# TGAC/KAT

Hardware: AMD Instinct MI355X
Metric: k-mers/sec (whole node) for kat comp reads-vs-assembly k=27 (higher is better)
Workload: dtype u64

## Files before the change

### kat_amd/csrc/kg_count.hip

```cpp
#include "kg_host.hpp"
#include "kg_ingest.hpp"
#include "kg_kernels.hpp"
#include "kg_partition.hpp"
#include "kg_partition_wide.hpp"
#include "kg_wide.hpp"

#include <condition_variable>
#include <deque>
#include <mutex>
#include <thread>


static const uint64_t g_test_sweep_thr = hook("KATGPU_TEST_SWEEP_THR") ? strtoull(hook("KATGPU_TEST_SWEEP_THR"), nullptr, 10) : 0;
static const uint64_t g_test_max_starts = hook("KATGPU_TEST_MAX_STARTS") ? strtoull(hook("KATGPU_TEST_MAX_STARTS"), nullptr, 10) : 0;

static int maybe_sweep(katgpu_table* t, uint64_t next_starts) {
    katgpu_ctx* c = t->ctx;
    if (t->dev().cbits) return KATGPU_OK;
    const uint64_t limit = g_test_sweep_thr ? 2 * g_test_sweep_thr - 1 : 0xFFFFFFFFULL;
    if (t->count_bound + t->unchecked_adds + next_starts <= limit) return KATGPU_OK;
    const uint32_t thr = g_test_sweep_thr ? (uint32_t)g_test_sweep_thr : 0x80000000u;
    unsigned long long* scratch = (unsigned long long*)&t->dev().ctrs[CTR_SCRATCH];
    HIPCHK(c, hipMemsetAsync(scratch, 0, sizeof(uint64_t), c->stream));
    {
        ScopedTimer tm(c, KATGPU_K_REGROW, t->dev().cap);
        hipLaunchKernelGGL(k_sweep, dim3(grid_for(c, t->dev().cap, 256, 8)), dim3(256), 0, c->stream, t->dev(), thr, scratch);
    }
    uint64_t mx = 0;
    HIPCHK(c, hipMemcpyAsync(&mx, scratch, sizeof mx, hipMemcpyDeviceToHost, c->stream));
    HIPCHK(c, hipStreamSynchronize(c->stream));
    t->count_bound = mx;
    t->unchecked_adds = 0;
    return KATGPU_OK;
}

static int launch_count(katgpu_table* t, const uint8_t* dev_bases, size_t n) {
    katgpu_ctx* c = t->ctx;
    if (n < t->dev().k) return KATGPU_OK;
    if (t->dev().keys_b) {
        const uint64_t n_chunks = (n + WIDE_CHUNK_STARTS - 1) / WIDE_CHUNK_STARTS;
        const int grid = (int)std::min<uint64_t>(n_chunks, (uint64_t)c->n_cu * 4);
        ScopedTimer tm(c, KATGPU_K_COUNT, n);
        if ((reinterpret_cast<uintptr_t>(dev_bases) & 15) == 0)
            hipLaunchKernelGGL((k_count<true, true>), dim3(grid), dim3(COUNT_BLOCK), 0, c->stream, t->dev(), dev_bases, (uint64_t)n, n_chunks);
        else
            hipLaunchKernelGGL((k_count<false, true>), dim3(grid), dim3(COUNT_BLOCK), 0, c->stream, t->dev(), dev_bases, (uint64_t)n, n_chunks);
        HIPCHK(c, hipGetLastError());
        return KATGPU_OK;
    }
    int src = maybe_sweep(t, n);
    if (src) return src;
    t->unchecked_adds += n;
    const uint64_t n_chunks = (n + CHUNK_STARTS - 1) / CHUNK_STARTS;
    const int grid = (int)std::min<uint64_t>(n_chunks, (uint64_t)c->n_cu * c->count_blocks_per_cu);
    ScopedTimer tm(c, KATGPU_K_COUNT, n);
    if ((reinterpret_cast<uintptr_t>(dev_bases) & 15) == 0)
        hipLaunchKernelGGL(k_count<true>, dim3(grid), dim3(COUNT_BLOCK), 0, c->stream, t->dev(), dev_bases, (uint64_t)n, n_chunks);
    else
        hipLaunchKernelGGL(k_count<false>, dim3(grid), dim3(COUNT_BLOCK), 0, c->stream, t->dev(), dev_bases, (uint64_t)n, n_chunks);
    HIPCHK(c, hipGetLastError());
    return KATGPU_OK;
}



static const uint64_t g_part_min_starts = getenv("KATGPU_PART_MIN_STARTS") ? strtoull(getenv("KATGPU_PART_MIN_STARTS"), nullptr, 10) : (32ULL << 20);
static const uint64_t g_test_round_items = hook("KATGPU_TEST_ROUND_ITEMS") ? strtoull(hook("KATGPU_TEST_ROUND_ITEMS"), nullptr, 10) : 0;
static const double g_arena_fraction = getenv("KATGPU_ARENA_FRACTION") ? std::min(0.95, std::max(0.05, atof(getenv("KATGPU_ARENA_FRACTION")))) : 0.85;
static const uint32_t g_p1_wgs = hook("KATGPU_P1_WGS") ? std::max<uint32_t>(1, (uint32_t)strtoul(hook("KATGPU_P1_WGS"), nullptr, 10)) : 3;
static const uint32_t g_test_l1_cpb = hook("KATGPU_TEST_L1_CPB") ? (uint32_t)strtoul(hook("KATGPU_TEST_L1_CPB"), nullptr, 10) : 0;
static const bool g_l1_lean = hook_u64("KATGPU_L1_LEAN", 1) != 0;
static const uint32_t g_l1_fast = hook("KATGPU_L1_FAST") ? (uint32_t)strtoul(hook("KATGPU_L1_FAST"), nullptr, 10) : 1;
static const uint32_t g_p2_fast = hook("KATGPU_P2_FAST") ? (uint32_t)strtoul(hook("KATGPU_P2_FAST"), nullptr, 10) : 1;
static const uint64_t g_test_p2_ovf_cap = hook("KATGPU_TEST_P2_OVF_CAP") ? strtoull(hook("KATGPU_TEST_P2_OVF_CAP"), nullptr, 10) : 0;
static const uint32_t g_test_spill_mod = hook("KATGPU_TEST_SPILL_MOD") ? (uint32_t)strtoul(hook("KATGPU_TEST_SPILL_MOD"), nullptr, 10) : 0;
static const uint64_t g_test_ap_seg = hook_u64("KATGPU_TEST_AP_SEG", 0) & ~3ULL;
static const uint32_t g_apply_per_cu = (uint32_t)hook_u64("KATGPU_APPLY_PER_CU", 0);
static const bool g_l1b_stamp = hook_u64("KATGPU_L1B_STAMP", 0) != 0;
static const bool g_p2x_stamp = hook_u64("KATGPU_P2X_STAMP", 0) != 0;
static const bool g_p2_stamp = hook_u64("KATGPU_P2_STAMP", 0) != 0;
static const bool g_apply_stamp = hook_u64("KATGPU_APPLY_STAMP", 0) != 0;

static bool part_geometry(const DevTable& d, PartGeom* g) {
    g->R = d.n_regions; g->S = d.region_slots; g->P1 = d.p1; g->P2 = d.p2; g->l2 = d.l2;
    g->b_lo = 0; g->b_hi = d.p1;
    g->pl = place_make(d.k, d.p1, d.n1, d.l2);
    g->hb = l2_hi_bytes(g->pl.rb);
    g->hb1 = l2_hi_bytes(g->pl.n1);
    g->cbits = d.cbits;
    if (d.cbits && g->hb > 2) g->hb = 2;
    return d.k <= 32 && g->pl.rb <= 63  && g->P1 <= MAX_PARTS && g->P2 <= MAX_PARTS && g->S % 4 == 0 && g->S >= 64 && g->S <= AP2_MAX_SLOTS;
}
static double l2_items_per_l1_item(uint32_t hb) { return 1 + 1.0 / 16 + 2.0 * MAX_PARTS / l2_tile_items(hb); }
static const uint32_t g_test_pass_buckets = hook("KATGPU_TEST_PASS_BUCKETS") ? (uint32_t)strtoul(hook("KATGPU_TEST_PASS_BUCKETS"), nullptr, 10) : 0;
static uint32_t pass_buckets(uint32_t p1, uint32_t n_cu) {
    if (g_test_pass_buckets) return std::max<uint32_t>(1, std::min(p1, g_test_pass_buckets));
    return n_cu && p1 > n_cu && p1 % n_cu == 0 ? n_cu : p1;
}
static double arena_bytes_per_item(uint32_t hb, uint32_t passes) { return 8.0 * (1 + 1.0 / 24) + l2_bytes_per_item(hb) * (1 + 1.0 / 24) * l2_items_per_l1_item(hb) / passes + 0.25 + 0.02; }

static const bool g_test_grow_nomem = hook("KATGPU_TEST_GROW_NOMEM") != nullptr;

static void insert_keys(katgpu_table* t, const void* keys, uint64_t n, size_t key_bytes) {
    katgpu_ctx* c = t->ctx;
    ScopedTimer tm(c, KATGPU_K_COUNT, n);
    if (key_bytes == 16) hipLaunchKernelGGL(k_insert_keys_w, dim3(grid_for(c, n, 256, 6)), dim3(256), 0, c->stream, t->dev(), (const u64x2*)keys, n);
    else hipLaunchKernelGGL(k_insert_keys, dim3(grid_for(c, n, 256, 6)), dim3(256), 0, c->stream, t->dev(), (const uint64_t*)keys, n);
}
typedef std::vector<std::pair<const void*, uint64_t>> KeyLists;
static int grow_beside_arena(katgpu_table* t, uint64_t incoming, uint64_t min_cap, const KeyLists& stash, size_t key_bytes, bool* arena_lost) {
    uint64_t n_stash = 0;
    for (auto& l : stash) n_stash += l.second;
    katgpu_ctx* c = t->ctx;
    auto grow = [&]() -> int {
        if (min_cap > t->dev().cap) {
            if (t->disable_grow) return fail(c, KATGPU_ERR_TABLE_FULL, "Hash full");
            uint64_t nc = t->dev().cap; while (nc < min_cap) nc *= 2;
            return regrow(t, nc);
        }
        return ensure_room(t, incoming);
    };
    *arena_lost = false;
    int rc = g_test_grow_nomem ? KATGPU_ERR_NOMEM : grow();
    if (rc != KATGPU_ERR_NOMEM) return rc;
    (void)hipGetLastError();
    std::vector<uint8_t> host;
    if (n_stash) {
        try { host.resize(n_stash * key_bytes); } catch (...) { return fail(c, KATGPU_ERR_NOMEM, "no host memory to park %llu spilled k-mers", (unsigned long long)n_stash); }
        uint64_t at = 0;
        for (auto& l : stash) { HIPCHK(c, hipMemcpy(host.data() + at * key_bytes, l.first, l.second * key_bytes, hipMemcpyDeviceToHost)); at += l.second; }
    }
    HIPCHK(c, hipStreamSynchronize(c->stream));
    release_arena(c);
    *arena_lost = true;
    if (g_trace) fprintf(stderr, "[katgpu] growth beside the partition arena failed: arena released, %llu keys parked on the host\n", (unsigned long long)n_stash);
    rc = grow();
    if (rc) return rc;
    if (n_stash) {
        const size_t chunk = std::min<size_t>(n_stash, ((size_t)256 << 20) / key_bytes);
        uint8_t* d = nullptr;
        HIPCHK(c, pool_alloc(c, (void**)&d, chunk * key_bytes));
        for (size_t i = 0; i < n_stash && rc == KATGPU_OK; i += chunk) {
            const size_t m = std::min(chunk, (size_t)n_stash - i);
            if (hipMemcpyAsync(d, host.data() + i * key_bytes, m * key_bytes, hipMemcpyHostToDevice, c->stream) != hipSuccess) { rc = fail(c, KATGPU_ERR_DEVICE, "spill upload"); break; }
            insert_keys(t, d, m, key_bytes);
            if (hipStreamSynchronize(c->stream) != hipSuccess) rc = fail(c, KATGPU_ERR_DEVICE, "spill insert");
        }
        pool_release(c, d);
    }
    return rc;
}

static int ensure_arena(katgpu_ctx* c, size_t small_bytes, size_t item_bytes, size_t want_items, size_t want_bytes, const char* note, bool* usable) {
    *usable = false;
    if (c->arena_limit) want_bytes = std::min(want_bytes, std::max(c->arena_limit, small_bytes + item_bytes * ((size_t)64 << 20)));
    if (c->arena_bytes < want_bytes) {
        size_t free_b = 0, total_b = 0;
        HIPCHK(c, hipMemGetInfo(&free_b, &total_b));
        free_b += c->arena_bytes;
        const size_t bytes = std::min<size_t>(want_bytes, (size_t)(g_arena_fraction * (double)free_b));
        if (bytes > c->arena_bytes + c->arena_bytes / 2 || c->arena_bytes < small_bytes + item_bytes * std::min<size_t>(want_items, (size_t)64 << 20)) {
            if (c->arena) { HIPCHK(c, hipFree(c->arena)); c->arena = nullptr; c->arena_bytes = 0; }
            if (!g_test_round_items && bytes < small_bytes + item_bytes * ((size_t)1 << 20)) return KATGPU_OK;
            const double t_ar = now_ms();
            if (hipMalloc((void**)&c->arena, bytes) != hipSuccess) { (void)hipGetLastError(); c->arena = nullptr; return KATGPU_OK; }
            c->arena_bytes = bytes;
            if (g_trace) fprintf(stderr, "[katgpu +%.0f ms] partition arena of %.1f GB%s: %.0f ms\n", since_load(), bytes / 1e9, note, now_ms() - t_ar);
        }
    }
    *usable = true;
    return KATGPU_OK;
}
struct ArenaBusy { katgpu_ctx* c; explicit ArenaBusy(katgpu_ctx* c_) : c(c_) { c->arena_busy = true; } ~ArenaBusy() { c->arena_busy = false; } };
template <typename T> static T* carve(uint8_t*& a, size_t bytes) { T* p = (T*)a; a += align_up(bytes, 256); return p; }

constexpr size_t LDS_BYTES = 160 * 1024, LDS_GRANULE = 1280;
template <typename K, typename... Args>
static int launch_lds(katgpu_ctx* c, K kern, dim3 grid, dim3 block, size_t lds, size_t ceiling, Args... args) {
    if (!c->lds_attr.count(reinterpret_cast<const void*>(kern))) {
        HIPCHK(c, hipFuncSetAttribute(reinterpret_cast<const void*>(kern), hipFuncAttributeMaxDynamicSharedMemorySize, (int)ceiling));
        c->lds_attr.insert(reinterpret_cast<const void*>(kern));
    }
    hipLaunchKernelGGL(kern, grid, block, lds, c->stream, args...);
    return KATGPU_OK;
}

struct StampLine { const char* head; int n_shown, n_sum; const char* phase[9];  int digits; };
static const StampLine STAMPS_L1B = {"[katgpu] level-1 (blocks) stamps (wave 0 of every workgroup, cycles summed):", 9, 9,
    {" codes %.*f %%", "  blocks out %.*f %%", " (+ barrier %.*f %%)", "  sweep %.*f %%", " (+ %.*f %%)", "  per bucket %.*f %%", " (+ %.*f %%)", "  placing %.*f %%", " (+ %.*f %%)"}, 1};
static const StampLine STAMPS_P2X = {"[katgpu] level-2 (blocks in, blocks out) stamps (wave 0 of every workgroup, cycles summed):", 7, 9,
    {" wait for the tile %.*f %%", " (+ barrier %.*f %%)", "  ranking + blocks out %.*f %%", " (+ %.*f %%)", "  per sub-bucket %.*f %%", " (+ %.*f %%)", "  placing %.*f %%"}, 1};
static const StampLine STAMPS_P2 = {"[katgpu] level-2 stamps (lane 0 of every workgroup, cycles summed):", 5, 5,
    {" wait for the tile %.*f %%", "  digit + rank %.*f %%", "  scan %.*f %%", "  staging %.*f %%", "  copy-out %.*f %%"}, 0};
constexpr int STAMP_AT_APPLY = 8, STAMP_AT = 16;
template <typename Launch>
static int with_stamps(katgpu_ctx* c, unsigned long long* dev, int n, const StampLine* line, Launch launch) {
    unsigned long long st[10];
    HIPCHK(c, hipMemsetAsync(dev, 0, n * sizeof(unsigned long long), c->stream));
    int rc = launch(dev);
    if (rc) return rc;
    HIPCHK(c, hipMemcpyAsync(st, dev, n * sizeof(unsigned long long), hipMemcpyDeviceToHost, c->stream));
    HIPCHK(c, hipStreamSynchronize(c->stream));
    double tot = line ? 0 : (double)(st[0] + st[1] + st[3] + st[4]);
    if (!line && st[5])
        fprintf(stderr, "[katgpu] apply stamps (wave 0 of every workgroup, cycles summed): fill %.3g (%.0f %%)  walk %.3g (%.0f %%; drains %.0f %% of the walk)  barrier + sweep %.3g (%.0f %%)  write-back %.3g (%.0f %%); %llu regions, %.1f chunks per wave and region, %.0f cycles per region\n",
                (double)st[0], 100 * st[0] / tot, (double)st[1], 100 * st[1] / tot, 100.0 * st[2] / std::max(1.0, (double)st[1]), (double)st[3], 100 * st[3] / tot, (double)st[4], 100 * st[4] / tot, st[5], (double)st[6] / st[5], tot / st[5]);
    if (!line || !st[n - 1]) return KATGPU_OK;
    for (int i = 0; i < line->n_sum; ++i) tot += (double)st[i];
    char buf[768];
    int at = snprintf(buf, sizeof buf, "%s", line->head);
    for (int i = 0; i < line->n_shown; ++i) at += snprintf(buf + at, sizeof buf - at, line->phase[i], line->digits, 100 * st[i] / tot);
    fprintf(stderr, "%s; %llu tiles, %.0f cycles per tile\n", buf, st[n - 1], tot / st[n - 1]);
    return KATGPU_OK;
}

struct ApplyLaunch {
    katgpu_table* t; const PartGeom& g; const uint64_t* off2; const uint8_t* l2_buf; uint64_t* spill_buf; unsigned long long* spill_n; const uint32_t* run_len; const uint64_t* bucket_end;
    dim3 grid; size_t lds; uint32_t qcap; uint64_t seg_len; uint32_t zero_fill;
};
template <int B, int KP, int HB, bool INL, bool HK, bool PF, int NR, bool STAMP = false>
static int apply_pk(const ApplyLaunch& a) {
    return launch_lds(a.t->ctx, k_p3_apply_pk<B, KP, HB, INL, HK, PF, NR, STAMP>, a.grid, dim3(B), a.lds, LDS_BYTES - 256, a.t->dv, a.g, a.off2, a.l2_buf, a.spill_buf, a.spill_n, a.run_len, a.bucket_end,
                      a.qcap, a.seg_len, g_test_spill_mod, a.zero_fill);
}
template <int HB>
static int apply_pk_shape(const ApplyLaunch& a, uint32_t blk, bool fresh, bool hooked) {
    if (hooked) return apply_pk<1024, 5, HB, false, true, true, 3>(a);
    if (blk == 1024) return fresh ? apply_pk<1024, 5, HB, true, false, true, 3>(a) : apply_pk<1024, 5, HB, false, false, true, 2>(a);
    if (a.g.S <= 4096) return fresh ? apply_pk<512, 4, HB, true, false, true, 3>(a) : apply_pk<512, 4, HB, false, false, true, 2>(a);
    if (HB == 1 && g_apply_stamp && !fresh)
        return with_stamps(a.t->ctx, a.spill_n + STAMP_AT_APPLY, 7, nullptr, [&](unsigned long long*) { return apply_pk<512, 10, 1, false, false, false, 2, true>(a); });
    return fresh ? apply_pk<512, 10, HB, true, false, false, 3>(a) : apply_pk<512, 10, HB, false, false, false, 2>(a);
}
template <int B, int KP, int HB, bool INL, int QC, bool HK>
static int apply_kv12(const ApplyLaunch& a) {
    return launch_lds(a.t->ctx, k_p3_apply2<B, KP, 4, 3, HB, false, INL, true, QC, HK>, a.grid, dim3(B), a.lds, LDS_BYTES - 256, a.t->dev(), a.g, a.off2, a.l2_buf, a.spill_buf, a.spill_n, a.run_len, a.bucket_end,
                      (unsigned long long*)nullptr, g_test_spill_mod, a.seg_len);
}
template <int HB>
static int apply_kv12_shape(const ApplyLaunch& a, uint32_t blk, bool big, bool fresh, bool hooked) {
    if (hooked) return apply_kv12<1024, 5, HB, false, AP2_QCAP_BIG, true>(a);
    if (blk == 512 && a.g.S <= 2048) return fresh ? apply_kv12<512, 2, HB, true, AP2_QCAP, false>(a) : apply_kv12<512, 2, HB, false, AP2_QCAP, false>(a);
    if (blk == 512) return fresh ? apply_kv12<512, 4, HB, true, AP2_QCAP, false>(a) : apply_kv12<512, 4, HB, false, AP2_QCAP, false>(a);
    if (big) return fresh ? apply_kv12<1024, 5, HB, true, AP2_QCAP_BIG, false>(a) : apply_kv12<1024, 5, HB, false, AP2_QCAP_BIG, false>(a);
    return fresh ? apply_kv12<1024, 4, HB, true, AP2_QCAP, false>(a) : apply_kv12<1024, 4, HB, false, AP2_QCAP, false>(a);
}
static int launch_apply(katgpu_table* t, const PartGeom& g, const uint64_t* off2, const uint8_t* l2_buf, uint64_t* spill_buf, unsigned long long* spill_n,
                        const uint32_t* run_len, const uint64_t* bucket_end) {
    katgpu_ctx* c = t->ctx;
    const uint32_t n_cu = (uint32_t)c->n_cu, regions = (g.b_hi - g.b_lo) * g.P2;
    const bool fresh = t->distinct == 0;
    const bool hooked = g_test_spill_mod != 0;
    ApplyLaunch a{t, g, off2, l2_buf, spill_buf, spill_n, run_len, bucket_end, dim3(1), 0, 0, 0, 0};
    int rc = KATGPU_OK;
    if (g.cbits) {
        const size_t region_b = (size_t)g.S * 8;
        auto room = [&](uint32_t wgs) -> long { return (long)(LDS_BYTES / wgs / LDS_GRANULE * LDS_GRANULE) - 64 - (long)region_b; };
        uint32_t per_cu = 4;
        auto min_q = [&](uint32_t wgs) -> long { return 8L * 8 * (wgs == 2 ? 72 : 96); };
        while (per_cu > 1 && room(per_cu) < min_q(per_cu)) --per_cu;
        if (g_apply_per_cu) per_cu = std::min(per_cu, g_apply_per_cu);
        uint32_t blk = per_cu == 1 ? 1024 : 512;
        if (hooked) { blk = 1024; per_cu = 1; }
        per_cu = std::min<uint32_t>(per_cu, 2048 / blk);
        const uint32_t nw = blk / 64;
        while (per_cu > 1 && room(per_cu) < (long)(nw * 72 * 8)) --per_cu;
        a.qcap = (uint32_t)std::min<long>(256, room(per_cu) / (long)(nw * 8));
        if (a.qcap < 72) return fail(c, KATGPU_ERR_DEVICE, "a region of %u packed slots leaves no room for the apply kernel's queues", g.S);
        a.lds = region_b + (size_t)nw * a.qcap * 8;
        const uint64_t seg_cap = (pk_half(g.cbits) - 1) & ~3ULL;
        a.seg_len = g_test_ap_seg ? std::min<uint64_t>(g_test_ap_seg, seg_cap) : std::min<uint64_t>(AP2_SEGMENT, seg_cap);
        a.grid = dim3(std::min<uint32_t>(regions, n_cu * per_cu));
        const uint64_t r_lo = (uint64_t)g.b_lo * g.P2, r_hi = (uint64_t)g.b_hi * g.P2;
        if (t->zero_from != ~0ULL) { if (t->zero_from == r_lo) a.zero_fill = 1; else t->zero_rest(); }
        switch (g.hb) {
        case 0: rc = apply_pk_shape<0>(a, blk, fresh, hooked); break;
        case 1: rc = apply_pk_shape<1>(a, blk, fresh, hooked); break;
        case 2: rc = apply_pk_shape<2>(a, blk, fresh, hooked); break;
        default: return fail(c, KATGPU_ERR_DEVICE, "packed apply: item width %u", g.hb);
        }
        if (rc) return rc;
        HIPCHK(c, hipGetLastError());
        if (a.zero_fill) t->zero_from = r_hi >= t->dv.n_regions ? ~0ULL : r_hi;
        return KATGPU_OK;
    }
    const uint32_t blk = hooked ? 1024 : (g.S <= 4096 ? 512 : 1024);
    const bool big = g.S > 8192 || hooked;
    a.lds = (size_t)g.S * 12 + (size_t)(blk / 64) * (big ? AP2_QCAP_BIG : AP2_QCAP) * 12;
    const uint32_t per_cu = (uint32_t)std::max<size_t>(1, std::min<size_t>(LDS_BYTES / (a.lds + 512), 2048 / blk));
    a.grid = dim3(std::min<uint32_t>(regions, n_cu * per_cu));
    a.seg_len = g_test_ap_seg ? std::min<uint64_t>(g_test_ap_seg, AP2_SEGMENT) : AP2_SEGMENT;
    switch (g.hb) {
    case 0: rc = apply_kv12_shape<0>(a, blk, big, fresh, hooked); break;
    case 1: rc = apply_kv12_shape<1>(a, blk, big, fresh, hooked); break;
    case 2: rc = apply_kv12_shape<2>(a, blk, big, fresh, hooked); break;
    case 4: rc = apply_kv12_shape<4>(a, blk, big, fresh, hooked); break;
    }
    if (rc) return rc;
    HIPCHK(c, hipGetLastError());
    return KATGPU_OK;
}

constexpr size_t SEG_PAD = 64;
struct PartArena {
    uint32_t hb, passes; double per_item; size_t fixed_l1, small_bytes;
    uint32_t* hist1; uint64_t* offs; uint64_t* l1_off; uint64_t* off2; uint32_t* cnt2; uint64_t* bend; unsigned long long* spill_n; unsigned long long* ovf_n;
    uint8_t* l1_buf;
    uint8_t* l2_buf;
    uint64_t* ovf_buf; uint64_t ovf_cap;
    size_t round_items, l1_items, l2_items;
    PartArena(const PartGeom& g0, uint32_t W, uint32_t n_cu) : hb(g0.hb), passes(std::max<uint32_t>(1, g0.P1 / pass_buckets(g0.P1, n_cu))), per_item(arena_bytes_per_item(hb, passes)) {
        fixed_l1 = (size_t)W * MAX_PARTS * SEG_PAD;
        const size_t fixed_l2 = (size_t)((double)fixed_l1 * l2_items_per_l1_item(hb) / passes) + (size_t)MAX_PARTS * MAX_PARTS * P2_RUN_SLACK + 8192;
        small_bytes = align_up((size_t)W * MAX_PARTS * 4, 256) + align_up((size_t)W * MAX_PARTS * 8, 256) +
                      align_up((MAX_PARTS + 1) * 8, 256) + align_up(((size_t)MAX_PARTS * MAX_PARTS + 1) * 8, 256) +
                      align_up((size_t)MAX_PARTS * MAX_PARTS * 4, 256) + align_up((size_t)MAX_PARTS * 8, 256) + align_up((size_t)MAX_PARTS * 4, 256) + 256 +
                      (fixed_l1 + fixed_l2 + 4096) * 8 + 4096;
    }
    void carve_from(uint8_t* a, size_t arena_bytes, uint32_t W, size_t want_items) {
        hist1 = carve<uint32_t>(a, (size_t)W * MAX_PARTS * 4);
        offs = carve<uint64_t>(a, (size_t)W * MAX_PARTS * 8);
        l1_off = carve<uint64_t>(a, (MAX_PARTS + 1) * 8);
        off2 = carve<uint64_t>(a, ((size_t)MAX_PARTS * MAX_PARTS + 1) * 8);
        cnt2 = carve<uint32_t>(a, (size_t)MAX_PARTS * MAX_PARTS * 4);
        bend = carve<uint64_t>(a, (size_t)MAX_PARTS * 8);
        carve<uint32_t>(a, (size_t)MAX_PARTS * 4);
        spill_n = carve<unsigned long long>(a, 256);
        ovf_n = spill_n + 1;
        round_items = std::min<size_t>(want_items, (size_t)((double)(arena_bytes - small_bytes) / per_item));
        l1_items = (round_items + round_items / 24 + fixed_l1 + 15) & ~(size_t)15;
        l2_items = ((size_t)((double)l1_items * l2_items_per_l1_item(hb) / passes) + (size_t)MAX_PARTS * MAX_PARTS * P2_RUN_SLACK + 4096 + 11) / 12 * 12;
        l1_buf = a;
        l2_buf = l1_buf + l1_items * 8;
        ovf_buf = (uint64_t*)(l2_buf + align_up(l2_buffer_bytes(hb, l2_items), 16));
        ovf_cap = g_test_p2_ovf_cap ? g_test_p2_ovf_cap : round_items / 32 + 1024;
    }
};
static int restore_ones(katgpu_table* t) { katgpu_ctx* c = t->ctx; HIPCHK(c, hipMemcpyAsync(&t->dv.ctrs[CTR_ONES], &t->ones, sizeof(uint64_t), hipMemcpyHostToDevice, c->stream)); return KATGPU_OK; }
static int probe_items_per_start(katgpu_table* t, const PartGeom& g, const PartArena& A, uint32_t W, const uint8_t* p, size_t left, double* items_per_start) {
    katgpu_ctx* c = t->ctx;
    const size_t probe_m = std::min<size_t>(left, (size_t)64 << 20) / P1_TILE_STARTS * P1_TILE_STARTS;
    const uint64_t pt = probe_m / P1_TILE_STARTS, ptw = (pt + W - 1) / W;
    hipLaunchKernelGGL(k_p1v2_count, dim3(W), dim3(P1_BLOCK), 0, c->stream, t->dv, g, p, (uint64_t)(probe_m + t->dv.k - 1), pt, ptw, A.hist1);
    hipLaunchKernelGGL(k_p1_scan, dim3(1), dim3(PART_BLOCK), 0, c->stream, g, W, A.hist1, A.offs, A.l1_off);
    uint64_t probe_items = 0;
    HIPCHK(c, hipMemcpyAsync(&probe_items, &A.l1_off[g.P1], sizeof probe_items, hipMemcpyDeviceToHost, c->stream));
    HIPCHK(c, hipStreamSynchronize(c->stream));
    *items_per_start = std::max(0.05, (double)probe_items / (double)probe_m);
    return t->dv.k == 32 && !t->dv.canonical ? restore_ones(t) : KATGPU_OK;
}
static size_t round_starts(size_t left, size_t round_items, double items_per_start) {
    size_t m = left;
    if (m > round_items) m = std::min(m, (size_t)((double)round_items / items_per_start * 0.98));
    if (m < left) {
        const size_t rounds_left = (left + m - 1) / m;
        m = (left + rounds_left - 1) / rounds_left;
        m += P1_TILE_STARTS - m % P1_TILE_STARTS;
        m = std::min(m, left);
    }
    return m;
}

enum class L1Edition { Blocks, SegLean512, SegLean1024, SegPlain512, SegPlain1024, ExactLean, ExactPlain };
struct L1Plan {
    L1Edition edition; bool seg ; uint32_t wgs ; uint64_t n_tiles, tiles_per_wg;
    uint64_t seg_cap, cap_plain, stride64;
};
static L1Plan plan_level1(const PartGeom& g, uint32_t k, size_t m, uint64_t est_items, uint32_t W, uint32_t n_cu, size_t l1_items, bool seg_wanted) {
    const bool lean = g_l1_lean && lean_applies(k, g.pl.n1);
    const bool pb512 = g.P1 <= 512;
    const bool l1b = lean && pb512 && g.hb1 == 2;
    const uint64_t n_tiles = (m + P1_TILE_STARTS - 1) / P1_TILE_STARTS;
    L1Plan pl;
    pl.wgs = l1b ? n_cu : W;
    pl.n_tiles = l1b ? (m + L1B_TILE_STARTS - 1) / L1B_TILE_STARTS : n_tiles;
    uint64_t seg_cap = est_items / ((uint64_t)pl.wgs * g.P1);
    seg_cap += seg_cap / 24 + SEG_PAD;
    if (g_test_l1_cpb) seg_cap = std::min<uint64_t>(seg_cap, g_test_l1_cpb);
    if (l1b) seg_cap = (seg_cap + L1B_ITEMS - 1) / L1B_ITEMS * L1B_ITEMS;
    pl.cap_plain = seg_cap;
    if (!l1b && g.hb1 != 4 && !g_test_l1_cpb) seg_cap += std::min<uint64_t>(3 * seg_cap, 2 * ((pl.n_tiles + pl.wgs - 1) / pl.wgs));
    if (!l1b) seg_cap = (seg_cap + 3) & ~3ULL;
    pl.seg_cap = seg_cap;
    pl.stride64 = l1b ? align_up(8 * (uint64_t)pl.wgs * pl.cap_plain + 32, 64)
                      : std::max<uint64_t>(8 * (uint64_t)pl.wgs * pl.cap_plain, (uint64_t)(4 + g.hb1) * pl.wgs * seg_cap) + 32;
    pl.seg = seg_wanted && pl.stride64 * g.P1 <= (uint64_t)l1_items * 8 &&
             seg_cap < (1u << 24) && pl.stride64 <= 0xFFFFFFFFULL ;
    if (pl.seg) pl.edition = l1b ? L1Edition::Blocks : lean ? (pb512 ? L1Edition::SegLean512 : L1Edition::SegLean1024) : (pb512 ? L1Edition::SegPlain512 : L1Edition::SegPlain1024);
    else { pl.edition = lean ? L1Edition::ExactLean : L1Edition::ExactPlain; pl.wgs = W; pl.n_tiles = n_tiles; }
    pl.tiles_per_wg = (pl.n_tiles + pl.wgs - 1) / pl.wgs;
    return pl;
}
static int launch_l1_scatter(katgpu_table* t, const PartGeom& g, const L1Plan& l1, const PartArena& A, const uint8_t* p, uint64_t nb) {
    katgpu_ctx* c = t->ctx;
    auto blocks = [&](auto kern, unsigned long long* stamps) {
        return launch_lds(c, kern, dim3(l1.wgs), dim3(L1B_THREADS), sizeof(P1BLds), sizeof(P1BLds), t->dv, g, p, nb, l1.n_tiles, l1.tiles_per_wg,
                          A.l1_buf, (uint32_t)(l1.seg_cap / L1B_ITEMS), (uint32_t)l1.stride64, A.ovf_buf, A.ovf_n, A.ovf_cap, stamps);
    };
    auto segmented = [&](auto kern) {
        hipLaunchKernelGGL(kern, dim3(l1.wgs), dim3(P1_BLOCK), 0, c->stream, t->dv, g, p, nb, l1.n_tiles, l1.tiles_per_wg, (const uint64_t*)nullptr, (const uint64_t*)nullptr, A.l1_buf,
                           (uint32_t)l1.seg_cap, (uint32_t)l1.stride64, (uint32_t)l1.cap_plain, A.ovf_buf, A.ovf_n, A.ovf_cap);
        return KATGPU_OK;
    };
    auto exact = [&](auto kern) {
        hipLaunchKernelGGL(kern, dim3(l1.wgs), dim3(P1_BLOCK), 0, c->stream, t->dv, g, p, nb, l1.n_tiles, l1.tiles_per_wg, (const uint64_t*)A.offs, (const uint64_t*)A.l1_off, A.l1_buf,
                           0u, 0u, 0u, (uint64_t*)nullptr, (unsigned long long*)nullptr, (uint64_t)0);
        return KATGPU_OK;
    };
    switch (l1.edition) {
    case L1Edition::Blocks:
        if (!g_l1b_stamp) return blocks(k_p1b_scatter<false>, nullptr);
        return with_stamps(c, A.spill_n + STAMP_AT, 10, &STAMPS_L1B, [&](unsigned long long* st) { return blocks(k_p1b_scatter<true>, st); });
    case L1Edition::SegLean512:   return segmented(k_p1v2_scatter<true, true, 512>);
    case L1Edition::SegLean1024:  return segmented(k_p1v2_scatter<true, true, MAX_PARTS>);
    case L1Edition::SegPlain512:  return segmented(k_p1v2_scatter<true, false, 512>);
    case L1Edition::SegPlain1024: return segmented(k_p1v2_scatter<true, false, MAX_PARTS>);
    case L1Edition::ExactLean:    return exact(k_p1v2_scatter<false, true, MAX_PARTS>);
    case L1Edition::ExactPlain:   return exact(k_p1v2_scatter<false, false, MAX_PARTS>);
    }
    return KATGPU_OK;
}
static int level1(katgpu_table* t, const PartGeom& g, const L1Plan& l1, const PartArena& A, const uint8_t* p, size_t m, double items_per_start, uint64_t* items) {
    katgpu_ctx* c = t->ctx;
    const uint64_t nb = m + t->dv.k - 1;
    if (l1.seg) {
        int rc;
        { ScopedTimer tm(c, KATGPU_K_PART_L1S, *items); rc = launch_l1_scatter(t, g, l1, A, p, nb); }
        if (!rc && g_trace) fprintf(stderr, "[katgpu] partition round (segmented level 1%s): %zu starts, ~%llu items, %llu k-mers per segment (arena %.1f GB)\n", l1.edition == L1Edition::Blocks ? ", blocks of ten" : "", m,
                                    (unsigned long long)*items, (unsigned long long)l1.seg_cap, c->arena_bytes / 1e9);
        return rc;
    }
    {
        ScopedTimer tm(c, KATGPU_K_PART_L1, m);
        hipLaunchKernelGGL(k_p1v2_count, dim3(l1.wgs), dim3(P1_BLOCK), 0, c->stream, t->dv, g, p, nb, l1.n_tiles, l1.tiles_per_wg, A.hist1);
        hipLaunchKernelGGL(k_p1_scan, dim3(1), dim3(PART_BLOCK), 0, c->stream, g, l1.wgs, A.hist1, A.offs, A.l1_off);
    }
    HIPCHK(c, hipMemcpyAsync(items, &A.l1_off[g.P1], sizeof *items, hipMemcpyDeviceToHost, c->stream));
    HIPCHK(c, hipStreamSynchronize(c->stream));
    if (g_trace) fprintf(stderr, "[katgpu] partition round: %zu starts -> %llu items (buffer %zu items, arena %.1f GB, ratio %.3f)\n", m, (unsigned long long)*items, A.round_items, c->arena_bytes / 1e9, items_per_start);
    if (*items > A.round_items) return t->dv.k == 32 && !t->dv.canonical ? restore_ones(t) : KATGPU_OK;
    if (!*items) return KATGPU_OK;
    ScopedTimer tm(c, KATGPU_K_PART_L1S, *items);
    return launch_l1_scatter(t, g, l1, A, p, nb);
}

enum class L1Items { Groups , WideGroups , Blocks  };
struct L2Pass { katgpu_ctx* c; const PartGeom& g; const PartArena& A; uint32_t grid; L1Items src; uint64_t seg_slots; };
template <typename K>
static int p2_one_pass(const L2Pass& x, K kern, size_t lds, unsigned long long* stamps = nullptr) {
    return launch_lds(x.c, kern, dim3(x.grid), dim3(PART_BLOCK), lds, lds, x.g, x.A.l1_off, x.A.l1_buf, x.A.l2_buf, x.A.off2, x.A.cnt2, x.A.ovf_buf, x.A.ovf_n, x.A.ovf_cap, x.seg_slots, stamps);
}
template <typename K>
static int p2_exact(const L2Pass& x, K kern, size_t lds) {
    return launch_lds(x.c, kern, dim3(x.grid), dim3(PART_BLOCK), lds, lds, x.g, x.A.l1_off, x.A.l1_buf, x.A.l2_buf, x.A.off2, x.seg_slots, x.A.bend);
}
template <int HB>
static int launch_l2_hb(const L2Pass& x, bool one_pass) {
    constexpr size_t lds_e = sizeof(P2Lds<HB>), lds_f = sizeof(typename P2FastLds<HB>::type);
    unsigned long long* const stamps = x.A.spill_n + STAMP_AT;
    switch (x.src) {
    case L1Items::Blocks:
        if constexpr (HB == 4) break;
        else if (!one_pass) return p2_exact(x, k_p2<HB, false, true>, lds_e);
        else if constexpr (HB != 1) return p2_one_pass(x, k_p2_fast<HB, false, false, true>, lds_f);
        else if (!g_p2x_stamp) return p2_one_pass(x, k_p2x_fast<false>, sizeof(P2XLds));
        else return with_stamps(x.c, stamps, 10, &STAMPS_P2X, [&](unsigned long long* st) { return p2_one_pass(x, k_p2x_fast<true>, sizeof(P2XLds), st); });
    case L1Items::WideGroups: return one_pass ? p2_one_pass(x, k_p2_fast<HB, true>, lds_f) : p2_exact(x, k_p2<HB, true>, lds_e);
    case L1Items::Groups:
        if constexpr (HB == 1) if (one_pass && g_p2_stamp) return with_stamps(x.c, stamps, 6, &STAMPS_P2, [&](unsigned long long* st) { return p2_one_pass(x, k_p2_fast<1, false, true>, lds_f, st); });
        return one_pass ? p2_one_pass(x, k_p2_fast<HB, false>, lds_f) : p2_exact(x, k_p2<HB, false>, lds_e);
    }
    return fail(x.c, KATGPU_ERR_DEVICE, "level 2 from blocked level-1 items: item width %u", x.g.hb);
}
static int launch_l2(const L2Pass& x, bool one_pass) {
    switch (x.g.hb) {
    case 0: return launch_l2_hb<0>(x, one_pass);
    case 1: return launch_l2_hb<1>(x, one_pass);
    case 2: return launch_l2_hb<2>(x, one_pass);
    case 4: return launch_l2_hb<4>(x, one_pass);
    }
    return fail(x.c, KATGPU_ERR_DEVICE, "level 2: item width %u", x.g.hb);
}
enum class L2Next { UseCnt2 , Exact , FallBackExact ,
                    RedoRound  };
static int read_overflow(katgpu_table* t, const PartArena& A, bool seg, bool tried_fast, unsigned long long ovf_l1, const unsigned long long* ovf_before, unsigned long long* overflowed, L2Next* next) {
    katgpu_ctx* c = t->ctx;
    HIPCHK(c, hipMemcpyAsync(overflowed, A.ovf_n, sizeof *overflowed, hipMemcpyDeviceToHost, c->stream));
    HIPCHK(c, hipStreamSynchronize(c->stream));
    if (seg && ovf_l1 > A.ovf_cap) {
        if (g_trace) fprintf(stderr, "[katgpu] segmented level 1: %llu k-mers beyond their segments (list holds %llu): exact level 1 from here on\n", ovf_l1, (unsigned long long)A.ovf_cap);
        *next = L2Next::RedoRound;
        return restore_ones(t);
// ... 582 lines not shown
```

### kat_amd/csrc/kg_l1_blocks.hpp

```cpp
#pragma once

namespace kg {

constexpr uint32_t L1B_ITEMS = 10, L1B_BYTES = 64;
constexpr int L1B_THREADS = 1024;
constexpr int L1B_TILE_BYTES = L1B_THREADS * PART_ITEMS;
constexpr int L1B_TILE_STARTS = L1B_TILE_BYTES - CHUNK_OVERLAP;
constexpr int L1B_LANES_WITH_STARTS = L1B_TILE_STARTS / PART_ITEMS;
constexpr uint32_t L1B_PB = 512;
constexpr uint32_t L1B_POOL = 1712;

struct P1BLds {
    uint32_t hist[L1B_PB + 64];
    uint2 gb[L1B_PB + 64];
    uint32_t where[L1B_POOL];
    uint32_t wave_tot[L1B_THREADS / 64];
    uint32_t code[L1B_THREADS + 2];
    uint16_t bad[L1B_THREADS + 2];
    __attribute__((aligned(16))) uint32_t img[(L1B_PB + L1B_POOL) * 16];
};
static_assert(sizeof(P1BLds) <= 160 * 1024 - 1280, "one workgroup per CU");

__device__ __forceinline__ uint32_t l1b_lo_at(uint32_t B, uint32_t s) { return B + 3 * (s >> 1) + (s & 1); }
__device__ __forceinline__ uint32_t l1b_hi_at(uint32_t B, uint32_t s) { return 2 * (B + 3 * (s >> 1) + 2) + (s & 1); }
__device__ __host__ __forceinline__ uint64_t l1b_item_lo(uint64_t i) { const uint64_t blk = i / L1B_ITEMS; const uint32_t s = (uint32_t)(i - blk * L1B_ITEMS); return blk * L1B_BYTES + 12 * (s >> 1) + 4 * (s & 1); }
__device__ __host__ __forceinline__ uint64_t l1b_item_hi(uint64_t i) { const uint64_t blk = i / L1B_ITEMS; const uint32_t s = (uint32_t)(i - blk * L1B_ITEMS); return blk * L1B_BYTES + 12 * (s >> 1) + 8 + 2 * (s & 1); }

template <bool STAMP = false >
__global__ void __launch_bounds__(L1B_THREADS)
k_p1b_scatter(DevTable t, PartGeom g, const uint8_t* __restrict__ bases, uint64_t n, uint64_t n_tiles, uint64_t tiles_per_wg,
              uint8_t* __restrict__ l1_buf, uint32_t segb , uint32_t bucket_stride ,
              uint64_t* __restrict__ ovf_buf, unsigned long long* __restrict__ ovf_n, uint64_t ovf_cap, unsigned long long* __restrict__ stamps) {
    constexpr uint32_t PB = L1B_PB;
    unsigned long long st[10] = {0, 0, 0, 0, 0, 0, 0, 0, 0, 0}, tq = 0;
    auto stamp = [&](int i) { if (STAMP) { const unsigned long long x = (unsigned long long)clock64(); st[i] += x - tq; tq = x; } };
    extern __shared__ __attribute__((aligned(16))) unsigned char lds_raw[];
    P1BLds& L = *reinterpret_cast<P1BLds*>(lds_raw);
    const uint32_t tid = threadIdx.x, P = g.P1, k = t.k;
    uint16_t* const img16 = reinterpret_cast<uint16_t*>(L.img);
    uint8_t* const seg0 = l1_buf + (uint64_t)blockIdx.x * segb * L1B_BYTES;
    const LeanGeom lg = lean_geom(k, t.canonical != 0, g.pl.n1);
    auto overflow = [&](uint32_t b, uint32_t lo, uint32_t hi) {
        const unsigned long long at = atomicAdd(ovf_n, 1ULL);
        if (at < ovf_cap) ovf_buf[at] = place_key_r1(b, ((uint64_t)hi << 32) | lo, g.pl);
    };
    if (tid < PB + 64) { L.hist[tid] = 0; L.gb[tid] = uint2{0u, 0u}; }
    if (tid < PB) L.img[tid * 16 + 15] = 0;
    const uint64_t t0 = (uint64_t)blockIdx.x * tiles_per_wg, t1 = min(t0 + tiles_per_wg, n_tiles);
    uint32_t n_out = 0;
    uint32_t tid_o = tid;
    constexpr int OUT_STEPS = (L1B_POOL + L1B_THREADS / 4 - 1) / (L1B_THREADS / 4);
    static_assert(OUT_STEPS <= PART_ITEMS / 2, "a step per pair of the sweep's k-mers");
    const uint32_t stride_b = bucket_stride >> 6;
    struct OutStep { u32x4 v; uint32_t where; };
    auto out_read = [&](int it, OutStep& o) {
        asm volatile("" : "+v"(tid_o));
        const uint32_t s = min((tid_o >> 2) + (uint32_t)it * (L1B_THREADS / 4), L1B_POOL - 1);
        o.where = L.where[s];
        o.v = *reinterpret_cast<const u32x4*>(&L.img[(PB + s) * 16 + (tid_o & 3) * 4]);
    };
    auto out_store = [&](int it, const OutStep& o) {
        asm volatile("" : "+v"(tid_o));
        if ((tid_o >> 2) + (uint32_t)it * (L1B_THREADS / 4) < n_out)
            *reinterpret_cast<u32x4*>(seg0 + (((uint64_t)o.where << 6) | ((tid_o & 3) * 16))) = o.v;
    };
    auto issue = [&](uint64_t tile_i) -> u32x4 {
        const uint64_t off = tile_i * L1B_TILE_STARTS + (uint64_t)tid_o * PART_ITEMS;
        return *reinterpret_cast<const u32x4*>(bases + (off + PART_ITEMS <= n ? off : 0));
    };
    u32x4 raw = issue(t0 < t1 ? t0 : 0);
    for (uint64_t tile = t0; tile < t1; ++tile) {
        if (STAMP) tq = (unsigned long long)clock64();
        asm volatile("" : "+v"(raw.x), "+v"(raw.y), "+v"(raw.z), "+v"(raw.w));
        {
            uint32_t w4[4] = {raw.x, raw.y, raw.z, raw.w}, code, bad;
            if (tile * L1B_TILE_STARTS + L1B_TILE_BYTES > n) p1_tile_fix(bases, n, tile * L1B_TILE_STARTS, raw, w4);
            encode16(w4, code, bad);
            L.code[tid] = code;
            L.bad[tid] = (uint16_t)bad;
            if (tid < 2) { L.code[L1B_THREADS + tid] = 0; L.bad[L1B_THREADS + tid] = 0xFFFF; }
        }
        stamp(0);
        asm volatile("" : "+v"(tid_o));
        raw = issue(tile + 1 < t1 ? tile + 1 : tile);
        stamp(1);
        lds_barrier();
        stamp(2);
        uint32_t lo[PART_ITEMS], hs[PART_ITEMS], rk2[PART_ITEMS / 2];
        const uint32_t v16 = tid < L1B_LANES_WITH_STARTS ? lean_valid16(L.bad[tid], L.bad[tid + 1], L.bad[tid + 2], k) : 0u;
        {
            LeanWin w{L.code[tid], L.code[tid + 1], L.code[tid + 2], 0, 0};
            uint32_t f_hi, f_lo;
            lean_fwd(w, lg, f_hi, f_lo);
            { const uint64_t rc0 = kmer_revcomp(((uint64_t)f_hi << 32) | f_lo, k); w.rc_hi = (uint32_t)(rc0 >> 32); w.rc_lo = (uint32_t)rc0; }
            const uint32_t dump = PB + (tid & 63);
            OutStep o;
#pragma unroll
            for (int j = 0; j < PART_ITEMS; ++j) {
                if (j % 2 == 0 && j / 2 < OUT_STEPS) out_read(j / 2, o);
                if (j) { lean_step(w); lean_fwd(w, lg, f_hi, f_lo); lean_rc_roll(w, lg, f_lo); }
                uint32_t key_hi, key_lo;
                bool took_rc;
                const uint32_t b = lean_digit1(w, lg, g.pl, f_hi, f_lo, key_hi, key_lo, took_rc);
                const bool ok = (v16 & (0x8000u >> j)) != 0;
                const uint32_t sel = ok ? b : dump;
                const uint32_t r = atomicAdd(&L.hist[sel], 1u);
                if (j & 1) rk2[j >> 1] |= r << 16; else rk2[j >> 1] = r;
                lo[j] = key_lo;
                hs[j] = (key_hi & lg.mask_lhi) | (sel << 16);
                if (j % 2 == 1 && j / 2 < OUT_STEPS) out_store(j / 2, o);
            }
        }
        stamp(3);
        lds_barrier();
        stamp(4);
        asm volatile("" : "+v"(tid_o));
        {
            uint32_t want = 0, avail = 0, nblk = 0, cur = 0, cn_old = 0;
            if (tid < P) {
                avail = L.hist[tid_o];
                const uint32_t w15 = L.img[tid_o * 16 + 15];
                cur = w15 & 0x0FFFFFFFu; cn_old = w15 >> 28;
                nblk = __umulhi(avail, 0xCCCCCCCDu) >> 3;
                want = min(nblk, segb > cur ? segb - cur : 0u);
            }
            const uint32_t lane = tid_o & 63, wave = tid_o >> 6;
            const uint32_t inc = wave_inclusive_scan(want);
            if (lane == 63) L.wave_tot[wave] = inc;
            lds_barrier();
            const uint32_t sc = wave_inclusive_scan(lane < L1B_THREADS / 64 ? L.wave_tot[lane] : 0u);
            const uint32_t wv = (uint32_t)__builtin_amdgcn_readfirstlane((int)wave);
            const uint32_t excl = (wv ? lane_value(sc, (int)wv - 1) : 0u) + inc - want;
            { const uint32_t tot = lane_value(sc, L1B_THREADS / 64 - 1); n_out = tot < L1B_POOL ? tot : L1B_POOL; }
            if (tid < P) {
                const uint32_t nst = excl < L1B_POOL ? min(want, L1B_POOL - excl) : 0u;
                const bool stuck = nblk != 0 && nst == 0;
                L.gb[tid_o] = uint2{(L1B_ITEMS * nst) | ((stuck ? 0xFFFFu : L1B_ITEMS * nblk) << 16), PB + excl};
                if (nst) {
                    const u32x4* src = reinterpret_cast<const u32x4*>(&L.img[tid_o * 16]);
                    u32x4* dst = reinterpret_cast<u32x4*>(&L.img[(PB + excl) * 16]);
                    const u32x4 a0 = src[0], a1 = src[1], a2 = src[2], a3 = src[3];
                    dst[0] = a0; dst[1] = a1; dst[2] = a2; dst[3] = a3;
                    const uint32_t first = tid_o * stride_b + cur;
                    for (uint32_t q = 0; q < nst; ++q) L.where[excl + q] = first + q;
                }
                const uint32_t cn = stuck ? cn_old : avail - L1B_ITEMS * nblk;
                L.img[tid_o * 16 + 15] = (cur + nst) | (cn << 28);
                L.hist[tid_o] = cn;
            } else if (tid < PB + 64) L.hist[tid_o] = 0;
        }
        stamp(5);
        lds_barrier();
        stamp(6);
        {
            uint32_t lostm = 0;
            constexpr int SB = 4;
#pragma unroll
            for (int j0 = 0; j0 < PART_ITEMS; j0 += SB) {
                uint2 G[SB];
#pragma unroll
                for (int u = 0; u < SB; ++u) G[u] = L.gb[hs[j0 + u] >> 16];
#pragma unroll
                for (int u = 0; u < SB; ++u) asm volatile("" : "+v"(G[u].x), "+v"(G[u].y));
#pragma unroll
                for (int u = 0; u < SB; ++u) {
                    const int j = j0 + u;
                    const bool ok = (v16 & (0x8000u >> j)) != 0;
                    const uint32_t v = (rk2[j >> 1] >> (16 * (j & 1))) & 0xFFFFu, lf = G[u].x >> 16;
                    const uint32_t q = __umulhi(v, 0xCCCCCCCDu) >> 3;
                    uint32_t s = v - L1B_ITEMS * q, B_p = G[u].y + q;
                    asm volatile("" : "+v"(s), "+v"(B_p));
                    const bool placed = v < (G[u].x & 0xFFFFu), later = v >= lf;
                    const uint32_t B = later ? hs[j] >> 16 : B_p, odd = s & 1u;
                    const uint32_t lo_at = (B << 6) + 6u * s - 2u * odd;
                    if (ok && (placed || later)) {
                        *reinterpret_cast<uint32_t*>(reinterpret_cast<unsigned char*>(L.img) + lo_at) = lo[j];
                        *reinterpret_cast<uint16_t*>(reinterpret_cast<unsigned char*>(L.img) + lo_at + 8u - 2u * odd) = (uint16_t)hs[j];
                    }
                    lostm |= (ok && !placed && !later) ? 1u << j : 0u;
                }
            }
            if (__any(lostm != 0)) {
#pragma unroll
                for (int j = 0; j < PART_ITEMS; ++j) if (lostm >> j & 1) overflow(hs[j] >> 16, lo[j], hs[j] & 0xFFFFu);
            }
        }
        stamp(7);
        lds_barrier();
        stamp(8);
        if (STAMP) st[9] += 1;
    }
    if (STAMP && tid == 0 && stamps) for (int i = 0; i < 10; ++i) atomicAdd(&stamps[i], st[i]);
#pragma unroll
    for (int it = 0; it < OUT_STEPS; ++it) { OutStep o; out_read(it, o); out_store(it, o); }
    lds_barrier();
    if (tid < P) {
        const uint32_t w15 = L.img[tid * 16 + 15], cur = w15 & 0x0FFFFFFFu, cn = w15 >> 28;
        L.img[tid * 16 + 15] = cur;
        const bool room = cur < segb;
        if (cn && !room) {
            for (uint32_t s = 0; s < cn; ++s) overflow(tid, L.img[l1b_lo_at(tid * 16, s)], img16[l1b_hi_at(tid * 16, s)]);
        }
        if (cn && room) for (uint32_t s = cn; s < L1B_ITEMS; ++s) { L.img[l1b_lo_at(tid * 16, s)] = 0xFFFFFFFFu; img16[l1b_hi_at(tid * 16, s)] = 0xFFFFu; }
        L.gb[tid].x = cn && room ? 1u : 0u;
    }
    lds_barrier();
    for (uint32_t qi = tid; qi < 4 * P; qi += L1B_THREADS) {
        const uint32_t b = qi >> 2, w = qi & 3;
        const uint32_t cur = L.img[b * 16 + 15];
        u32x4 v = *reinterpret_cast<const u32x4*>(&L.img[b * 16 + 4 * w]);
        if (w == 3) v.w = 0xFFFFFFFFu;
        if (L.gb[b].x) *reinterpret_cast<u32x4*>(seg0 + ((uint64_t)b * bucket_stride + ((uint64_t)cur << 6) + 16 * w)) = v;
    }
    lds_barrier();
    {
        const uint32_t wave = tid >> 6, lane = tid & 63;
        for (uint32_t b = wave; b < P; b += L1B_THREADS / 64) {
            const uint32_t from = L.img[b * 16 + 15] + L.gb[b].x;
            uint8_t* seg = seg0 + (uint64_t)b * bucket_stride;
            for (uint32_t q = from * 4 + lane; q < segb * 4; q += 64) *reinterpret_cast<u32x4*>(seg + (uint64_t)q * 16) = u32x4{0xFFFFFFFFu, 0xFFFFFFFFu, 0xFFFFFFFFu, 0xFFFFFFFFu};
        }
    }
}

}
```

Baseline: 100.1 billion.

## Split level-1 scatter workgroup into two half-tile groups that alternate phases

The 1024-thread level-1 scatter workgroup is split into two 512-thread groups. Each group processes alternate half-size tiles with its own code/bad buffers and its own half of the output pool, and the second group is offset by three barriers so one group's encode and sweep overlap the other's per-bucket step. The aim is to hide the serial per-bucket scan and pool copy behind the other group's work instead of idling most threads. The cost is smaller tiles with more overlap overhead, a halved staging pool per group, and a delicate barrier-count balance, including extra barriers at the end based on tile parity.

```diff
diff --git a/kat_amd/csrc/kg_count.hip b/kat_amd/csrc/kg_count.hip
--- a/kat_amd/csrc/kg_count.hip
+++ b/kat_amd/csrc/kg_count.hip
@@ -186,8 +186,8 @@
 }
 
 struct StampLine { const char* head; int n_shown, n_sum; const char* phase[9];  int digits; };
-static const StampLine STAMPS_L1B = {"[katgpu] level-1 (blocks) stamps (wave 0 of every workgroup, cycles summed):", 9, 9,
-    {" codes %.*f %%", "  blocks out %.*f %%", " (+ barrier %.*f %%)", "  sweep %.*f %%", " (+ %.*f %%)", "  per bucket %.*f %%", " (+ %.*f %%)", "  placing %.*f %%", " (+ %.*f %%)"}, 1};
+static const StampLine STAMPS_L1B = {"[katgpu] level-1 (blocks, half-tiles) stamps (wave 0 of every workgroup = group X, cycles summed):", 9, 9,
+    {" codes %.*f %%", "  next request %.*f %%", " (+ the other group's per-bucket step %.*f %%)", "  sweep + blocks out %.*f %%", " (+ %.*f %%)", "  per bucket %.*f %%", " (+ %.*f %%)", "  placing %.*f %%", " (+ %.*f %%)"}, 1};
 static const StampLine STAMPS_P2X = {"[katgpu] level-2 (blocks in, blocks out) stamps (wave 0 of every workgroup, cycles summed):", 7, 9,
     {" wait for the tile %.*f %%", " (+ barrier %.*f %%)", "  ranking + blocks out %.*f %%", " (+ %.*f %%)", "  per sub-bucket %.*f %%", " (+ %.*f %%)", "  placing %.*f %%"}, 1};
 static const StampLine STAMPS_P2 = {"[katgpu] level-2 stamps (lane 0 of every workgroup, cycles summed):", 5, 5,
diff --git a/kat_amd/csrc/kg_l1_blocks.hpp b/kat_amd/csrc/kg_l1_blocks.hpp
--- a/kat_amd/csrc/kg_l1_blocks.hpp
+++ b/kat_amd/csrc/kg_l1_blocks.hpp
@@ -3,21 +3,22 @@
 namespace kg {
 
 constexpr uint32_t L1B_ITEMS = 10, L1B_BYTES = 64;
-constexpr int L1B_THREADS = 1024;
-constexpr int L1B_TILE_BYTES = L1B_THREADS * PART_ITEMS;
+constexpr int L1B_THREADS = 1024, L1B_GROUP = L1B_THREADS / 2;
+constexpr int L1B_TILE_BYTES = L1B_GROUP * PART_ITEMS;
 constexpr int L1B_TILE_STARTS = L1B_TILE_BYTES - CHUNK_OVERLAP;
 constexpr int L1B_LANES_WITH_STARTS = L1B_TILE_STARTS / PART_ITEMS;
 constexpr uint32_t L1B_PB = 512;
-constexpr uint32_t L1B_POOL = 1712;
+constexpr uint32_t L1B_POOL = 856;
+static_assert(L1B_PB == (uint32_t)L1B_GROUP, "thread b of the half-tile's owner is bucket b");
 
 struct P1BLds {
     uint32_t hist[L1B_PB + 64];
     uint2 gb[L1B_PB + 64];
-    uint32_t where[L1B_POOL];
-    uint32_t wave_tot[L1B_THREADS / 64];
-    uint32_t code[L1B_THREADS + 2];
-    uint16_t bad[L1B_THREADS + 2];
-    __attribute__((aligned(16))) uint32_t img[(L1B_PB + L1B_POOL) * 16];
+    uint32_t where[2 * L1B_POOL];
+    uint32_t wave_tot[L1B_GROUP / 64];
+    uint32_t code[2][L1B_GROUP + 2];
+    uint16_t bad[2][L1B_GROUP + 2];
+    __attribute__((aligned(16))) uint32_t img[(L1B_PB + 2 * L1B_POOL) * 16];
 };
 static_assert(sizeof(P1BLds) <= 160 * 1024 - 1280, "one workgroup per CU");
 
@@ -28,7 +29,7 @@
 
 template <bool STAMP = false >
 __global__ void __launch_bounds__(L1B_THREADS)
-k_p1b_scatter(DevTable t, PartGeom g, const uint8_t* __restrict__ bases, uint64_t n, uint64_t n_tiles, uint64_t tiles_per_wg,
+k_p1b_scatter(DevTable t, PartGeom g, const uint8_t* __restrict__ bases, uint64_t n, uint64_t n_tiles , uint64_t tiles_per_wg,
               uint8_t* __restrict__ l1_buf, uint32_t segb , uint32_t bucket_stride ,
               uint64_t* __restrict__ ovf_buf, unsigned long long* __restrict__ ovf_n, uint64_t ovf_cap, unsigned long long* __restrict__ stamps) {
     constexpr uint32_t PB = L1B_PB;
@@ -37,6 +38,8 @@
     extern __shared__ __attribute__((aligned(16))) unsigned char lds_raw[];
     P1BLds& L = *reinterpret_cast<P1BLds*>(lds_raw);
     const uint32_t tid = threadIdx.x, P = g.P1, k = t.k;
+    const uint32_t grp = (uint32_t)__builtin_amdgcn_readfirstlane((int)(tid / L1B_GROUP));
+    const uint32_t pool0 = grp * L1B_POOL;
     uint16_t* const img16 = reinterpret_cast<uint16_t*>(L.img);
     uint8_t* const seg0 = l1_buf + (uint64_t)blockIdx.x * segb * L1B_BYTES;
     const LeanGeom lg = lean_geom(k, t.canonical != 0, g.pl.n1);
@@ -47,49 +50,65 @@
     if (tid < PB + 64) { L.hist[tid] = 0; L.gb[tid] = uint2{0u, 0u}; }
     if (tid < PB) L.img[tid * 16 + 15] = 0;
     const uint64_t t0 = (uint64_t)blockIdx.x * tiles_per_wg, t1 = min(t0 + tiles_per_wg, n_tiles);
+    const uint32_t n_all = t0 < t1 ? (uint32_t)(t1 - t0) : 0u, n_mine = (n_all + 1 - grp) / 2;
     uint32_t n_out = 0;
-    uint32_t tid_o = tid;
-    constexpr int OUT_STEPS = (L1B_POOL + L1B_THREADS / 4 - 1) / (L1B_THREADS / 4);
+    uint32_t tg_o = tid % L1B_GROUP;
+    constexpr int OUT_STEPS = (L1B_POOL + L1B_GROUP / 4 - 1) / (L1B_GROUP / 4);
     static_assert(OUT_STEPS <= PART_ITEMS / 2, "a step per pair of the sweep's k-mers");
     const uint32_t stride_b = bucket_stride >> 6;
     struct OutStep { u32x4 v; uint32_t where; };
     auto out_read = [&](int it, OutStep& o) {
-        asm volatile("" : "+v"(tid_o));
-        const uint32_t s = min((tid_o >> 2) + (uint32_t)it * (L1B_THREADS / 4), L1B_POOL - 1);
+        asm volatile("" : "+v"(tg_o));
+        const uint32_t s = pool0 + min((tg_o >> 2) + (uint32_t)it * (L1B_GROUP / 4), L1B_POOL - 1);
         o.where = L.where[s];
-        o.v = *reinterpret_cast<const u32x4*>(&L.img[(PB + s) * 16 + (tid_o & 3) * 4]);
+        o.v = *reinterpret_cast<const u32x4*>(&L.img[(PB + s) * 16 + (tg_o & 3) * 4]);
     };
     auto out_store = [&](int it, const OutStep& o) {
-        asm volatile("" : "+v"(tid_o));
-        if ((tid_o >> 2) + (uint32_t)it * (L1B_THREADS / 4) < n_out)
-            *reinterpret_cast<u32x4*>(seg0 + (((uint64_t)o.where << 6) | ((tid_o & 3) * 16))) = o.v;
+        asm volatile("" : "+v"(tg_o));
+        if ((tg_o >> 2) + (uint32_t)it * (L1B_GROUP / 4) < n_out)
+            *reinterpret_cast<u32x4*>(seg0 + (((uint64_t)o.where << 6) | ((tg_o & 3) * 16))) = o.v;
     };
     auto issue = [&](uint64_t tile_i) -> u32x4 {
-        const uint64_t off = tile_i * L1B_TILE_STARTS + (uint64_t)tid_o * PART_ITEMS;
+        const uint64_t off = tile_i * L1B_TILE_STARTS + (uint64_t)tg_o * PART_ITEMS;
         return *reinterpret_cast<const u32x4*>(bases + (off + PART_ITEMS <= n ? off : 0));
     };
-    u32x4 raw = issue(t0 < t1 ? t0 : 0);
-    for (uint64_t tile = t0; tile < t1; ++tile) {
+    u32x4 raw = issue(n_mine ? t0 + grp : 0);
+    if (grp) { lds_barrier(); lds_barrier(); lds_barrier(); }
+    for (uint32_t m = 0; m < n_mine; ++m) {
+        const uint64_t tile = t0 + grp + 2 * (uint64_t)m;
         if (STAMP) tq = (unsigned long long)clock64();
         asm volatile("" : "+v"(raw.x), "+v"(raw.y), "+v"(raw.z), "+v"(raw.w));
+        asm volatile("" : "+v"(tg_o));
         {
             uint32_t w4[4] = {raw.x, raw.y, raw.z, raw.w}, code, bad;
-            if (tile * L1B_TILE_STARTS + L1B_TILE_BYTES > n) p1_tile_fix(bases, n, tile * L1B_TILE_STARTS, raw, w4);
+            if (tile * L1B_TILE_STARTS + L1B_TILE_BYTES > n) {
+                const uint64_t off = tile * L1B_TILE_STARTS + (uint64_t)tg_o * PART_ITEMS;
+                if (off + PART_ITEMS > n) {
+#pragma unroll
+                    for (int q = 0; q < 4; ++q) {
+                        uint32_t x = 0;
+#pragma unroll
+                        for (int b = 0; b < 4; ++b) { const uint64_t i = off + q * 4 + b; x |= (i < n ? (uint32_t)bases[i] : (uint32_t)'N') << (8 * b); }
+                        w4[q] = x;
+                    }
+                }
+            }
             encode16(w4, code, bad);
-            L.code[tid] = code;
-            L.bad[tid] = (uint16_t)bad;
-            if (tid < 2) { L.code[L1B_THREADS + tid] = 0; L.bad[L1B_THREADS + tid] = 0xFFFF; }
+            L.code[grp][tg_o] = code;
+            L.bad[grp][tg_o] = (uint16_t)bad;
+            if (tg_o < 2) { L.code[grp][L1B_GROUP + tg_o] = 0; L.bad[grp][L1B_GROUP + tg_o] = 0xFFFF; }
         }
         stamp(0);
-        asm volatile("" : "+v"(tid_o));
-        raw = issue(tile + 1 < t1 ? tile + 1 : tile);
+        asm volatile("" : "+v"(tg_o));
+        raw = issue(m + 1 < n_mine ? tile + 2 : tile);
         stamp(1);
+        lds_barrier();
         lds_barrier();
         stamp(2);
         uint32_t lo[PART_ITEMS], hs[PART_ITEMS], rk2[PART_ITEMS / 2];
-        const uint32_t v16 = tid < L1B_LANES_WITH_STARTS ? lean_valid16(L.bad[tid], L.bad[tid + 1], L.bad[tid + 2], k) : 0u;
-        {
-            LeanWin w{L.code[tid], L.code[tid + 1], L.code[tid + 2], 0, 0};
+        const uint32_t v16 = tg_o < L1B_LANES_WITH_STARTS ? lean_valid16(L.bad[grp][tg_o], L.bad[grp][tg_o + 1], L.bad[grp][tg_o + 2], k) : 0u;
+        {
+            LeanWin w{L.code[grp][tg_o], L.code[grp][tg_o + 1], L.code[grp][tg_o + 2], 0, 0};
             uint32_t f_hi, f_lo;
             lean_fwd(w, lg, f_hi, f_lo);
             { const uint64_t rc0 = kmer_revcomp(((uint64_t)f_hi << 32) | f_lo, k); w.rc_hi = (uint32_t)(rc0 >> 32); w.rc_lo = (uint32_t)rc0; }
@@ -114,40 +133,41 @@
         stamp(3);
         lds_barrier();
         stamp(4);
-        asm volatile("" : "+v"(tid_o));
+        asm volatile("" : "+v"(tg_o));
         {
             uint32_t want = 0, avail = 0, nblk = 0, cur = 0, cn_old = 0;
-            if (tid < P) {
-                avail = L.hist[tid_o];
-                const uint32_t w15 = L.img[tid_o * 16 + 15];
+            if (tg_o < P) {
+                avail = L.hist[tg_o];
+                const uint32_t w15 = L.img[tg_o * 16 + 15];
                 cur = w15 & 0x0FFFFFFFu; cn_old = w15 >> 28;
                 nblk = __umulhi(avail, 0xCCCCCCCDu) >> 3;
                 want = min(nblk, segb > cur ? segb - cur : 0u);
             }
-            const uint32_t lane = tid_o & 63, wave = tid_o >> 6;
+            const uint32_t lane = tg_o & 63, wave = tg_o >> 6;
             const uint32_t inc = wave_inclusive_scan(want);
             if (lane == 63) L.wave_tot[wave] = inc;
             lds_barrier();
-            const uint32_t sc = wave_inclusive_scan(lane < L1B_THREADS / 64 ? L.wave_tot[lane] : 0u);
+            const uint32_t sc = wave_inclusive_scan(lane < L1B_GROUP / 64 ? L.wave_tot[lane] : 0u);
             const uint32_t wv = (uint32_t)__builtin_amdgcn_readfirstlane((int)wave);
             const uint32_t excl = (wv ? lane_value(sc, (int)wv - 1) : 0u) + inc - want;
-            { const uint32_t tot = lane_value(sc, L1B_THREADS / 64 - 1); n_out = tot < L1B_POOL ? tot : L1B_POOL; }
-            if (tid < P) {
+            { const uint32_t tot = lane_value(sc, L1B_GROUP / 64 - 1); n_out = tot < L1B_POOL ? tot : L1B_POOL; }
+            if (tg_o < P) {
                 const uint32_t nst = excl < L1B_POOL ? min(want, L1B_POOL - excl) : 0u;
                 const bool stuck = nblk != 0 && nst == 0;
-                L.gb[tid_o] = uint2{(L1B_ITEMS * nst) | ((stuck ? 0xFFFFu : L1B_ITEMS * nblk) << 16), PB + excl};
+                L.gb[tg_o] = uint2{(L1B_ITEMS * nst) | ((stuck ? 0xFFFFu : L1B_ITEMS * nblk) << 16), PB + pool0 + excl};
                 if (nst) {
-                    const u32x4* src = reinterpret_cast<const u32x4*>(&L.img[tid_o * 16]);
-                    u32x4* dst = reinterpret_cast<u32x4*>(&L.img[(PB + excl) * 16]);
+                    const u32x4* src = reinterpret_cast<const u32x4*>(&L.img[tg_o * 16]);
+                    u32x4* dst = reinterpret_cast<u32x4*>(&L.img[(PB + pool0 + excl) * 16]);
                     const u32x4 a0 = src[0], a1 = src[1], a2 = src[2], a3 = src[3];
                     dst[0] = a0; dst[1] = a1; dst[2] = a2; dst[3] = a3;
-                    const uint32_t first = tid_o * stride_b + cur;
-                    for (uint32_t q = 0; q < nst; ++q) L.where[excl + q] = first + q;
+                    const uint32_t first = tg_o * stride_b + cur;
+                    for (uint32_t q = 0; q < nst; ++q) L.where[pool0 + excl + q] = first + q;
                 }
                 const uint32_t cn = stuck ? cn_old : avail - L1B_ITEMS * nblk;
-                L.img[tid_o * 16 + 15] = (cur + nst) | (cn << 28);
-                L.hist[tid_o] = cn;
-            } else if (tid < PB + 64) L.hist[tid_o] = 0;
+                L.img[tg_o * 16 + 15] = (cur + nst) | (cn << 28);
+                L.hist[tg_o] = cn;
+            } else L.hist[tg_o] = 0;
+            if (tg_o < 64) L.hist[PB + tg_o] = 0;
         }
         stamp(5);
         lds_barrier();
@@ -190,6 +210,7 @@
         stamp(8);
         if (STAMP) st[9] += 1;
     }
+    if ((n_all & 1u) == grp) { lds_barrier(); lds_barrier(); lds_barrier(); }
     if (STAMP && tid == 0 && stamps) for (int i = 0; i < 10; ++i) atomicAdd(&stamps[i], st[i]);
 #pragma unroll
     for (int it = 0; it < OUT_STEPS; ++it) { OutStep o; out_read(it, o); out_store(it, o); }
```

New measurement: 98.39 billion. -1.7%, worse.
